# spvkgn/vorbis-aotuv-lancer

Measured on AMD Instinct MI355X. Metric: realtime-stream-equivalents/node (44.1kHz stereo q5) + MDCT HBM GB/s, higher is better.
Workload: dtype f32

## Files before the change

vorbis_aotuv_lancer_amd/csrc/capi_frontend.cpp:

```cpp
#include <hip/hip_runtime.h>
#include <stdio.h>
#include <string.h>
#include <string>
#include <vector>

#include "vorbis_mi355x.h"
#include "setup_host.h"
#include "frontend.h"
#include "frontend_kernels.h"
#include "mdct_kernel.h"
#include "kernels.h"
#include "vbm_internal.h"

struct vbm_frontend {
    vbm_encoder *enc;
    vbm_setup_host *H;
    const vbm_setup *hs;
    int S, ch;
    vbm_fe_state f;
    std::vector<void *> allocs;
    vbm_fe_decision *d_dec = nullptr, *h_dec = nullptr;
    int *d_ids = nullptr, *d_begin = nullptr;
    int *h_ids = nullptr, *h_begin = nullptr;
    uint8_t *h_flags = nullptr;
    vbm_fe_job *d_jobs = nullptr, *h_jobs = nullptr;
    uint8_t *d_hold = nullptr, *h_hold = nullptr;
    bool hold_active = false;
    float *d_blocks = nullptr;
    int blocks_turn = 0, nblocks_bufs = 2;
    std::vector<int> pcm_current, W, started, ended;
    hipStream_t q = nullptr;
    hipEvent_t ev_in = nullptr, ev_out = nullptr;
    int lane0[4] = {0, 0, 0, 0}, lane_cap[4] = {0, 0, 0, 0}, lanes = 0;
    signed char *d_type = nullptr;
    int *d_slot = nullptr, *d_begin_lane = nullptr;
    unsigned long long *d_stats = nullptr;
    float *d_blocks_dev = nullptr;
    std::vector<long long> written;
    bool mirrors_stale = false;
    bool dirty = false;
    int pending_steps = 0;
};

template <typename T>
static int fe_alloc(vbm_frontend *fe, T **p, size_t count)
{
    hipError_t err = hipMalloc((void **)p, count * sizeof(T) + 256);
    if (err != hipSuccess) return vbm_set_hip_error(err, "hipMalloc(front end)");
    fe->allocs.push_back(*p);
// ... 57 lines not shown
    f.base_max = (int)(bs1 * (cap_blocks / 3));
    f.plane = (long)S * ch * f.cap;
    f.marks = (int)(f.cap / 64) + 8;
    int rc = 0;
#define A(field, type, count) do { type *p_; rc = fe_alloc<type>(fe, &p_, (count)); if (rc) { vbm_frontend_destroy(fe); return rc; } field = p_; } while (0)
    const size_t SC = (size_t)S * ch;
    A(f.pcm, float, (size_t)2 * f.plane);
    A(f.parity, int, S);
    A(f.base, int, S);
    A(f.overflow, int, 1);
    A(f.pcm_current, int, S); A(f.centerW, int, S); A(f.lW, int, S); A(f.W, int, S); A(f.nW, int, S);
    A(f.eofflag, int, S); A(f.preextrapolate, int, S);
    A(f.granulepos, long long, S); A(f.sequence, long long, S);
    A(f.ve_current, int, S); A(f.ve_cursor, int, S); A(f.ve_curmark, int, S); A(f.ve_stretch, int, S);
    A(f.ve_mark, int, (size_t)f.marks * S);
    A(f.ve_ampbuf, float, (size_t)16 * VBM_VE_AMP * SC);
    A(f.ve_ampptr, int, (size_t)16 * SC);
    A(f.ve_nearDC, float, (size_t)VBM_VE_NEARDC * SC);
    A(f.ve_nearacc, float, (size_t)2 * SC);
    A(f.ve_nearptr, int, SC);
    A(f.ve_first, int, S); A(f.ve_last, int, S);
    A(f.ve_spec, float, SC * VBM_FE_CHUNK * 64);
    A(fe->d_dec, vbm_fe_decision, S);
    A(fe->d_ids, int, S); A(fe->d_begin, int, S);
    fe->nblocks_bufs = vbm_encoder_workspaces(enc);
    A(fe->d_blocks, float, (size_t)fe->nblocks_bufs * SC * bs1);
    A(fe->d_hold, uint8_t, (size_t)S);
    if (hipHostMalloc((void **)&fe->h_hold, (size_t)S, hipHostMallocDefault) != hipSuccess) {
        vbm_frontend_destroy(fe);
        g_vbm_err = "hipHostMalloc(hold mask) failed";
// ... 31 lines not shown
    if (!fe) return VBM_EINVAL;
    const vbm_fe_state &f = fe->f;
    const int S = fe->S, bs1 = fe->hs->blocksizes[1];
    const size_t SC = (size_t)S * fe->ch;
    hipError_t err = hipDeviceSynchronize();
    auto zero = [&](void *p, size_t bytes) { if (err == hipSuccess) err = hipMemset(p, 0, bytes); };
    zero(f.pcm, (size_t)2 * f.plane * sizeof(float));
    zero(f.parity, S * sizeof(int));
    zero(f.base, S * sizeof(int));
    zero(f.overflow, sizeof(int));
    zero(f.lW, S * sizeof(int)); zero(f.W, S * sizeof(int)); zero(f.nW, S * sizeof(int));
    zero(f.eofflag, S * sizeof(int)); zero(f.preextrapolate, S * sizeof(int));
    zero(f.granulepos, S * sizeof(long long));
    zero(f.ve_current, S * sizeof(int)); zero(f.ve_stretch, S * sizeof(int));
    zero(f.ve_mark, (size_t)f.marks * S * sizeof(int));
    zero(f.ve_ampbuf, (size_t)16 * VBM_VE_AMP * SC * sizeof(float));
    zero(f.ve_ampptr, (size_t)16 * SC * sizeof(int));
    zero(f.ve_nearDC, (size_t)VBM_VE_NEARDC * SC * sizeof(float));
    zero(f.ve_nearacc, 2 * SC * sizeof(float));
    zero(f.ve_nearptr, SC * sizeof(int));
    if (err != hipSuccess) return vbm_set_hip_error(err, "hipMemset(front end)");
    std::vector<int> half(S, bs1 / 2), minus1(S, -1);
    std::vector<long long> seq(S, 3);
    if ((err = hipMemcpy(f.pcm_current, half.data(), S * sizeof(int), hipMemcpyHostToDevice)) != hipSuccess ||
        (err = hipMemcpy(f.centerW, half.data(), S * sizeof(int), hipMemcpyHostToDevice)) != hipSuccess ||
        (err = hipMemcpy(f.ve_cursor, half.data(), S * sizeof(int), hipMemcpyHostToDevice)) != hipSuccess ||
        (err = hipMemcpy(f.ve_curmark, minus1.data(), S * sizeof(int), hipMemcpyHostToDevice)) != hipSuccess ||
        (err = hipMemcpy(f.sequence, seq.data(), S * sizeof(long long), hipMemcpyHostToDevice)) != hipSuccess)
        return vbm_set_hip_error(err, "hipMemcpy(front end init)");
    fe->pcm_current.assign(S, bs1 / 2);
// ... 305 lines not shown
    }
    if ((err = hipMemcpyAsync(fe->d_ids, fe->h_ids, total * sizeof(int), hipMemcpyHostToDevice, st)) != hipSuccess ||
        (err = hipMemcpyAsync(fe->d_begin, fe->h_begin, total * sizeof(int), hipMemcpyHostToDevice, st)) != hipSuccess)
        return vbm_set_hip_error(err, "hipMemcpyAsync(round lists)");

    {
        int rc = vbm_analysis_round_wait_workspace(fe->enc, fq);
        if (rc) return rc;
    }
    float *round_blocks = fe->d_blocks + (size_t)fe->blocks_turn * S * ch * bs1;
    fe->blocks_turn = (fe->blocks_turn + 1) % fe->nblocks_bufs;
    for (int m = 0; m < 4; m++) {
        if (!count[m]) continue;
        const int N = (m >> 1) ? bs1 : bs0;
        float *blocks = round_blocks + (size_t)offset[m] * ch * bs1;
        if (vbm_fe_launch_gather(&fe->f, fe->d_ids + offset[m], fe->d_begin + offset[m], count[m], N, blocks, nullptr, st))
            return VBM_EHIP;
    }
    vbm_debug_delay_point(VBM_DP_FE_FORK, st);
    {
        int rc = vbm_analysis_round_begin(fe->enc, count, fe->h_ids, fe->h_flags, round_blocks, d_packets, d_packet_bytes, fq);
        if (rc) return rc;
        if (!defer && (rc = vbm_analysis_round_join(fe->enc, stream))) return rc;
    }
    vbm_debug_delay_point(VBM_DP_FE_SHIFT, st);
    if (vbm_fe_launch_shift(&fe->f, fe->d_dec, st)) return VBM_EHIP;
    *nblocks = total;
    return VBM_OK;
}

extern "C" int vbm_frontend_encode_round(vbm_frontend *fe, uint8_t *d_packets, int *d_packet_bytes,
// ... 138 lines not shown
{
    if (!fe || nrounds < 1 || !d_packet_bytes || !d_info || !d_counts) return VBM_EINVAL;
    const vbm_setup *s = fe->hs;
    const vbm_setup *ds = vbm_setup_device(fe->H);
    const int S = fe->S, ch = fe->ch, bs0 = s->blocksizes[0], bs1 = s->blocksizes[1];
    const int maxb = vbm_encoder_max_packet_bytes(fe->enc);
    hipStream_t q = fe->q;
    hipError_t err;
    int rc = fe_enter(fe, stream);
    if (rc) return rc;
    vbm_debug_stamp(q, 1);
    if (!fe->lanes) {
        lane_layout(s, S, fe->lane0, fe->lane_cap, &fe->lanes);
        const size_t L = (size_t)fe->lanes;
#define A(field, type, count) do { type *p_; rc = fe_alloc<type>(fe, &p_, (count)); if (rc) return rc; field = p_; } while (0)
        A(fe->d_type, signed char, (size_t)S);
        A(fe->d_slot, int, (size_t)S);
        A(fe->d_begin_lane, int, L);
        A(fe->d_stats, unsigned long long, 8);
        A(fe->d_blocks_dev, float, (size_t)fe->nblocks_bufs * L * ch * bs1);
#undef A
        if ((err = hipDeviceSynchronize()) != hipSuccess) return vbm_set_hip_error(err, "hipDeviceSynchronize");
    }
    if (fe_evaluate_envelope(fe, q)) return VBM_EHIP;
    for (int r = 0; r < nrounds; r++) {
        int w, ws_lanes;
        int *d_sid, *counts_ws;
        uint8_t *d_wf;
        rc = vbm_encoder_device_round_open(fe->enc, q, &w, &d_sid, &d_wf, &ws_lanes, &counts_ws);
        if (rc) return rc;
        if (ws_lanes < fe->lanes) {
            g_vbm_err = "encoder workspace too small for rounds built on the device: create it with max_batch >= vbm_device_round_lanes()";
            return VBM_EINVAL;
        }
        float *blocks = fe->d_blocks_dev + (size_t)w * fe->lanes * ch * bs1;
        int *counts_r = d_counts + 4 * r;
        int *bytes_r = d_packet_bytes + (size_t)r * fe->lanes;
        int caps[4];
        for (int m = 0; m < 4; m++) caps[m] = fe->lane_cap[m];
        if (r > 0 && caps[2] > 0 && caps[3] > 2 * caps[2]) caps[3] = 2 * caps[2];
        vbm_fe_round R;
        for (int m = 0; m < 4; m++) { R.lane0[m] = fe->lane0[m]; R.cap[m] = caps[m]; }
        R.first_round = r == 0;
        R.count = counts_ws;
        R.slot = fe->d_slot;
        R.stream_id = d_sid;
        R.wflags = d_wf;
        R.begin = fe->d_begin_lane;
        R.info = d_info + (size_t)r * fe->lanes;
        R.stats = fe->d_stats;
        vbm_debug_delay_point(VBM_DP_DEV_PLAN, q);
        if (vbm_fe_launch_round_plan(&fe->f, ds, &R, fe->d_type, fe->d_dec, bytes_r, fe->lanes, q)) return VBM_EHIP;
        if ((err = hipMemcpyAsync(counts_r, counts_ws, 4 * sizeof(int), hipMemcpyDeviceToDevice, q)) != hipSuccess)
            return vbm_set_hip_error(err, "hipMemcpyAsync(counts)");
        for (int m = 0; m < 4; m++) {
            if (!caps[m]) continue;
            const int N = (m >> 1) ? bs1 : bs0;
            if (vbm_fe_launch_gather(&fe->f, d_sid + fe->lane0[m], fe->d_begin_lane + fe->lane0[m], caps[m], N,
                                     blocks + (size_t)fe->lane0[m] * ch * bs1, counts_ws + m, q))
                return VBM_EHIP;
        }
        vbm_debug_stamp(q, 2 + (r ? 1 : 0));
        rc = vbm_encoder_device_round_run(fe->enc, w, fe->lane0, caps, counts_ws, blocks,
                                          d_packets ? d_packets + (size_t)r * fe->lanes * maxb : nullptr, bytes_r, r == 0, q);
        if (rc) return rc;
        vbm_debug_delay_point(VBM_DP_FE_SHIFT, q);
        if (vbm_fe_launch_shift(&fe->f, fe->d_dec, q)) return VBM_EHIP;
    }
    vbm_debug_stamp(q, 4);
    fe->mirrors_stale = true;
    if (lazy == 2) return VBM_OK;
    return lazy ? vbm_analysis_round_join_lazy(fe->enc, stream) : vbm_analysis_round_join(fe->enc, stream);
}

extern "C" int vbm_frontend_round_types(vbm_frontend *fe, signed char *out, void *stream)
{
    if (!fe || !out || !fe->d_type) return VBM_EINVAL;
    hipError_t err = hipMemcpyAsync(out, fe->d_type, (size_t)fe->S, hipMemcpyDeviceToHost, (hipStream_t)stream);
    return err == hipSuccess ? VBM_OK : vbm_set_hip_error(err, "hipMemcpyAsync(round types)");
}

extern "C" int vbm_frontend_device_stats(vbm_frontend *fe, unsigned long long *out)
{
    if (!fe || !out) return VBM_EINVAL;
    for (int i = 0; i < 6; i++) out[i] = 0;
    hipError_t err;
    int ov = 0;
    if ((err = hipStreamSynchronize(fe->q)) != hipSuccess ||
        (err = hipMemcpy(&ov, fe->f.overflow, sizeof(int), hipMemcpyDeviceToHost)) != hipSuccess)
        return vbm_set_hip_error(err, "hipMemcpy(stats)");
    out[5] = (unsigned long long)ov;
    if (!fe->d_stats) return VBM_OK;
    if ((err = hipMemcpy(out, fe->d_stats, 5 * sizeof(unsigned long long), hipMemcpyDeviceToHost)) != hipSuccess)
        return vbm_set_hip_error(err, "hipMemcpy(stats)");
    return VBM_OK;
}

extern "C" int vbm_debug_poison_frontend(vbm_frontend *fe, int byte)
{
    if (!fe) return VBM_EINVAL;
    hipError_t err = hipDeviceSynchronize();
    if (err != hipSuccess) return vbm_set_hip_error(err, "hipDeviceSynchronize");
    const size_t SC = (size_t)fe->S * fe->ch, bs1 = (size_t)fe->hs->blocksizes[1];
    if ((err = hipMemset(fe->d_blocks, byte, (size_t)fe->nblocks_bufs * SC * bs1 * sizeof(float))) != hipSuccess ||
        (err = hipMemset(fe->f.ve_spec, byte, SC * VBM_FE_CHUNK * 64 * sizeof(float))) != hipSuccess ||
        (err = hipMemset(fe->d_ids, byte, (size_t)fe->S * sizeof(int))) != hipSuccess ||
        (err = hipMemset(fe->d_begin, byte, (size_t)fe->S * sizeof(int))) != hipSuccess ||
        (fe->d_blocks_dev && (err = hipMemset(fe->d_blocks_dev, byte, (size_t)fe->nblocks_bufs * fe->lanes * fe->ch * bs1 * sizeof(float))) != hipSuccess) ||
        (fe->d_begin_lane && (err = hipMemset(fe->d_begin_lane, byte, (size_t)fe->lanes * sizeof(int))) != hipSuccess))
        return vbm_set_hip_error(err, "hipMemset(poison)");
    err = hipDeviceSynchronize();
    return err == hipSuccess ? VBM_OK : vbm_set_hip_error(err, "hipDeviceSynchronize");
}

extern "C" int vbm_frontend_join(vbm_frontend *fe, void *stream)
{
    if (!fe) return VBM_EINVAL;
    return vbm_analysis_round_join(fe->enc, stream);
}
```

vorbis_aotuv_lancer_amd/csrc/frontend.h:

```cpp
#pragma once
#include <stdint.h>
#include "setup.h"
#include "vorbis_mi355x.h"

#define VBM_FE_CHUNK 32

struct vbm_fe_state {
    int S, ch;
    long cap;
    long plane;
    int marks;
    float *pcm;
    int *parity;
    int *base;
    int base_max;
    int *overflow;
    int *pcm_current, *centerW, *lW, *W, *nW, *eofflag, *preextrapolate;
    long long *granulepos, *sequence;
    int *ve_current, *ve_cursor, *ve_curmark, *ve_stretch;
    int *ve_mark;
    float *ve_ampbuf;
    int *ve_ampptr;
    float *ve_nearDC;
    float *ve_nearacc;
    int *ve_nearptr;
    int *ve_first, *ve_last;
    float *ve_spec;
};

struct vbm_fe_job {
    long long src;
    long long ch_stride;
    int stream, vals;
};

struct vbm_fe_decision {
    int ready;
    int lW, W, nW;
    int block_mode;
    int eos;
    int beginW;
    int movement;
    long long granulepos, sequence;
};

struct vbm_fe_round {
    int lane0[4], cap[4];
    int first_round;
    int *count;
    int *slot;
    int *stream_id;
    uint8_t *wflags;
    int *begin;
    vbm_packet_info *info;
    unsigned long long *stats;
};
```

vorbis_aotuv_lancer_amd/csrc/frontend_kernels.h:

```cpp
#pragma once
#include <hip/hip_runtime.h>
#include "frontend.h"

extern "C" {
int vbm_fe_launch_append(const vbm_fe_state *f, const float *d_src, int vals, float pre_amplitude, hipStream_t st);
int vbm_fe_launch_append_ids(const vbm_fe_state *f, const int *d_ids, int n, const float *d_src, int vals,
                             float pre_amplitude, long stream_stride, long ch_stride, int by_slot, hipStream_t st);
int vbm_fe_launch_append_ragged(const vbm_fe_state *f, const vbm_fe_job *d_jobs, int n, int max_vals, const float *d_src,
                                float pre_amplitude, hipStream_t st);
int vbm_fe_launch_restart(const vbm_fe_state *f, const int *d_ids, int n, int long_n, hipStream_t st);
int vbm_fe_launch_extrapolate(const vbm_fe_state *f, const int *d_ids, int nids, int mode, int long_n, hipStream_t st);
int vbm_fe_launch_ve_range(const vbm_fe_state *f, hipStream_t st);
int vbm_fe_launch_ve_filter(const vbm_fe_state *f, const vbm_setup *d_setup, int t0, hipStream_t st);
int vbm_fe_launch_decide(const vbm_fe_state *f, const vbm_setup *d_setup, vbm_fe_decision *d_out, const uint8_t *d_hold,
                         hipStream_t st);
int vbm_fe_launch_gather(const vbm_fe_state *f, const int *d_ids, const int *d_begin, int count, int N, float *d_dst,
                         const int *d_count, hipStream_t st);
int vbm_fe_launch_round_plan(const vbm_fe_state *f, const vbm_setup *d_setup, const vbm_fe_round *r, signed char *d_type,
                             vbm_fe_decision *d_dec, int *d_packet_bytes, int lanes, hipStream_t st);
int vbm_fe_launch_shift(const vbm_fe_state *f, const vbm_fe_decision *d_dec, hipStream_t st);
}
```

vorbis_aotuv_lancer_amd/csrc/frontend_kernels.hip:

```cpp
#include <hip/hip_runtime.h>
#include <stdint.h>
#include "batch.h"
#include "frontend.h"
#include "frontend_kernels.h"

namespace {

__device__ __forceinline__ float *chan_buf(const vbm_fe_state &f, int s, int c)
{
    return f.pcm + (long)f.parity[s] * f.plane + ((long)s * f.ch + c) * f.cap + f.base[s];
}

__device__ __forceinline__ bool fe_full(const vbm_fe_state &f, int s, int vals)
{
    return f.base[s] + f.pcm_current[s] + vals > f.cap;
}

__device__ __forceinline__ void fe_append_one(const vbm_fe_state &f, int s, int c, const float *in, int vals,
                                              float pre_amplitude)
{
    if (fe_full(f, s, vals)) return;
    float *dst = f.pcm + (long)f.parity[s] * f.plane + (long)(s * f.ch + c) * f.cap + f.base[s] + f.pcm_current[s];
    const int t0 = blockIdx.y * blockDim.x + threadIdx.x, step = gridDim.y * blockDim.x;
    if ((((uintptr_t)dst | (uintptr_t)in) & 15) == 0 && (vals & 3) == 0) {
// ... 68 lines not shown
    float *pcm = f.pcm + (long)f.parity[s] * f.plane + c * f.cap;
    for (int i = 0; i < long_n / 2; i++) pcm[i] = 0.f;
    for (int k = 0; k < VBM_VE_AMP; k++)
        for (int jb = 0; jb < 16; jb++) f.ve_ampbuf[((long)k * SC + c) * 16 + jb] = 0.f;
    for (int jb = 0; jb < 16; jb++) f.ve_ampptr[c * 16 + jb] = 0;
    for (int k = 0; k < VBM_VE_NEARDC; k++) f.ve_nearDC[(long)k * SC + c] = 0.f;
    f.ve_nearacc[c] = 0.f;
    f.ve_nearacc[SC + c] = 0.f;
    f.ve_nearptr[c] = 0;
    if (ci == 0) {
        f.base[s] = 0;
        f.pcm_current[s] = long_n / 2; f.centerW[s] = long_n / 2;
        f.lW[s] = 0; f.W[s] = 0; f.nW[s] = 0; f.eofflag[s] = 0; f.preextrapolate[s] = 0;
        f.granulepos[s] = 0; f.sequence[s] = 3;
        f.ve_current[s] = 0; f.ve_cursor[s] = long_n / 2; f.ve_curmark[s] = -1; f.ve_stretch[s] = 0;
        for (int k = 0; k < f.marks; k++) f.ve_mark[(long)k * f.S + s] = 0;
    }
}

template <int M, typename Acc>
__device__ void lpc_from_data(Acc data, float *lpci, int n)
{
    double aut[M + 1], lpc[M];
    double error, epsilon;
    int i, j;

    j = M + 1;
    while (j--) {
        double d = 0;
        for (i = j; i < n; i++) d += (double)data(i) * (double)data(i - j);
        aut[j] = d;
// ... 122 lines not shown
__global__ __launch_bounds__(64) void k_fe_ve_filter(vbm_fe_state f, const vbm_setup *__restrict__ setup, int t0)
{
    __shared__ float s_vec[4][32];
    extern __shared__ float s_ring[];
    const int grp = threadIdx.x >> 4, jb = threadIdx.x & 15;
    const int s = blockIdx.x * 4 + grp;
    if (s >= f.S) return;
    const vbm_envelope *ve = &setup->ve;
    const long SC = (long)f.S * f.ch;
    const int first = f.ve_first[s] + t0, last = f.ve_last[s];
    if (first >= last) return;
    const int ch = f.ch;
    const float minV = ve->minenergy;
    const float stretch_penalty = ve->stretch_penalty;
    int ve_stretch = f.ve_stretch[s];
    const int S = f.S;
    const bool band = jb < VBM_VE_BANDS;
    const int begin = band ? ve->band_begin[jb] : 0, end = band ? ve->band_end[jb] : 0;
    const float total = band ? ve->band_total[jb] : 0.f;
    const float pre_t = band ? ve->preecho_thresh[jb] : 0.f, post_t = band ? ve->postecho_thresh[jb] : 0.f;
    float bw[VBM_VE_MAXBAND];
#pragma unroll
    for (int i = 0; i < VBM_VE_MAXBAND; i++) bw[i] = band ? ve->band_window[jb][i] : 0.f;

    constexpr int PER_CH = VBM_VE_AMP * 16 + 16 + 16 + 4;
    float *R = s_ring + (size_t)grp * ch * PER_CH;
    for (int ci = 0; ci < ch; ci++) {
        const long c = (long)s * ch + ci;
        float *rc = R + ci * PER_CH;
#pragma unroll
        for (int k = 0; k < VBM_VE_AMP; k++) rc[k * 16 + jb] = f.ve_ampbuf[((long)k * SC + c) * 16 + jb];
// ... 130 lines not shown

            if (valmax > pre_t + penalty) ret |= 1 | 4;
            if (valmin < post_t - penalty) ret |= 2;
        }
        __builtin_amdgcn_fence(__ATOMIC_RELEASE, "wavefront");
        __builtin_amdgcn_wave_barrier();
        __builtin_amdgcn_fence(__ATOMIC_ACQUIRE, "wavefront");

        if (ci == ch - 1) {
            ret |= __builtin_amdgcn_update_dpp(0, ret, 0xB1, 0xf, 0xf, true);
            ret |= __builtin_amdgcn_update_dpp(0, ret, 0x4E, 0xf, 0xf, true);
            ret |= __builtin_amdgcn_update_dpp(0, ret, 0x141, 0xf, 0xf, true);
            ret |= __builtin_amdgcn_update_dpp(0, ret, 0x140, 0xf, 0xf, true);

            if (jb == 0) {
                f.ve_mark[(long)(j + VBM_VE_POST) * S + s] = 0;
                if (ret & 1) {
                    f.ve_mark[(long)j * S + s] = 1;
                    f.ve_mark[(long)(j + 1) * S + s] = 1;
                }
                if (ret & 2) {
                    f.ve_mark[(long)j * S + s] = 1;
                    if (j > 0) f.ve_mark[(long)(j - 1) * S + s] = 1;
                }
            }
            if (ret & 4) ve_stretch = -1;
        }
    }
    if (jb == 0) {
        f.ve_stretch[s] = ve_stretch;
        if (first + nsteps >= last) f.ve_current[s] = last * 64;
    }

    for (int ci = 0; ci < ch; ci++) {
        const long c = (long)s * ch + ci;
        const float *rc = R + ci * PER_CH;
#pragma unroll
        for (int k = 0; k < VBM_VE_AMP; k++) f.ve_ampbuf[((long)k * SC + c) * 16 + jb] = rc[k * 16 + jb];
// ... 8 lines not shown
    }
}

__device__ __forceinline__ vbm_fe_decision fe_no_decision()
{
    vbm_fe_decision d;
    d.ready = 0; d.lW = d.W = d.nW = 0; d.block_mode = 0; d.eos = 0; d.beginW = 0; d.movement = 0;
    d.granulepos = 0; d.sequence = 0;
    return d;
}

template <bool COMMIT>
__device__ __forceinline__ void fe_decide_one(const vbm_fe_state &f, const vbm_setup *__restrict__ setup, const int s,
                                              vbm_fe_decision &d)
{
    const int S = f.S;
    const int searchstep = 64;
    const int bs0 = setup->blocksizes[0], bs1 = setup->blocksizes[1];
    d = fe_no_decision();

    int W = f.W[s], lW = f.lW[s], nW = f.nW[s];
    int centerW = f.centerW[s], pcm_current = f.pcm_current[s], eofflag = f.eofflag[s];
    const int bsW = W ? bs1 : bs0;
    const int beginW = centerW - bsW / 2;

    if (!f.preextrapolate[s] || eofflag == -1) return;

    int bp = -1;
    int curmark;
    {
        const int ve_current = (pcm_current / searchstep - VBM_VE_WIN) * searchstep;
        if (COMMIT) f.ve_current[s] = ve_current;
        const int testW = centerW + bsW / 4 + bs1 / 2 + bs0 / 4;
        int j = f.ve_cursor[s];
        int cursor = j;
        curmark = f.ve_curmark[s];
        while (j < ve_current - searchstep) {
            if (j >= testW) { bp = 1; break; }
            cursor = j;
            if (f.ve_mark[(long)(j / searchstep) * S + s]) {
                if (j > centerW) {
                    curmark = j;
                    bp = (j >= testW) ? 1 : 0;
                    break;
                }
            }
            j += searchstep;
        }
        if (COMMIT) {
            f.ve_cursor[s] = cursor;
            f.ve_curmark[s] = curmark;
        }
    }

    if (bp == -1) {
// ... 12 lines not shown
    }

    d.ready = 1;
    d.lW = lW; d.W = W; d.nW = nW;
    int blocktype;
    if (W) {
        blocktype = (!lW || !nW) ? 0  : 1 ;
    } else {
        int b0 = centerW - bs0 / 4 - bs0 / 4;
        int e0 = centerW + bs0 / 4 + bs0 / 4;
        int marked = 0;
        if (curmark >= b0 && curmark < e0) marked = 1;
        else {
            const int first = b0 / searchstep, last = e0 / searchstep;
            for (int i = first; i < last; i++)
                if (f.ve_mark[(long)i * S + s]) { marked = 1; break; }
        }
        blocktype = marked ? 0  : 1 ;
    }
    d.block_mode = blocktype | (W << 1);
    if (!COMMIT) return;
    d.sequence = f.sequence[s]++;
    long long granulepos = f.granulepos[s];
    d.granulepos = granulepos;
    d.beginW = beginW;

    if (eofflag) {
        if (centerW >= eofflag) {
            f.eofflag[s] = -1;
            d.eos = 1;
            return;
        }
    }

    {
        const int new_centerNext = bs1 / 2;
        const int movementW = centerNext - new_centerNext;
        if (movementW > 0) {
            {
                int ve_current = f.ve_current[s];
                const int smallsize = ve_current / searchstep + VBM_VE_POST;
                const int smallshift = movementW / searchstep;
                for (int k = 0; k < smallsize - smallshift; k++)
                    f.ve_mark[(long)k * S + s] = f.ve_mark[(long)(k + smallshift) * S + s];
                f.ve_current[s] = ve_current - movementW;
                int cm = f.ve_curmark[s];
                if (cm >= 0) f.ve_curmark[s] = cm - movementW;
                f.ve_cursor[s] -= movementW;
            }
            pcm_current -= movementW;
            f.pcm_current[s] = pcm_current;
            d.movement = movementW;

            f.lW[s] = W;
            f.W[s] = nW;
            f.centerW[s] = new_centerNext;
            centerW = new_centerNext;

            if (eofflag) {
// ... 9 lines not shown
        }
    }
}

__global__ void k_fe_decide(vbm_fe_state f, const vbm_setup *__restrict__ setup, vbm_fe_decision *__restrict__ out,
                            const uint8_t *__restrict__ hold)
{
    const int s = blockIdx.x * blockDim.x + threadIdx.x;
    if (s >= f.S) return;
    vbm_fe_decision d;
    if (hold && hold[s]) d = fe_no_decision();
    else fe_decide_one<true>(f, setup, s, d);
    out[s] = d;
}

__global__ void k_fe_classify(vbm_fe_state f, const vbm_setup *__restrict__ setup, signed char *__restrict__ type)
{
    const int s = blockIdx.x * blockDim.x + threadIdx.x;
    if (s >= f.S) return;
    vbm_fe_decision d;
    d.ready = 0;
    fe_decide_one<false>(f, setup, s, d);
    type[s] = d.ready ? (signed char)(d.block_mode & 3) : (signed char)-1;
}

__global__ __launch_bounds__(1024) void k_fe_plan(vbm_fe_round r, const signed char *__restrict__ type, int S)
{
    __shared__ int s_part[16][4];
    __shared__ int s_carry[4];
    const int lane = threadIdx.x & 63, wave = threadIdx.x >> 6;
    if (threadIdx.x < 4) s_carry[threadIdx.x] = 0;
    __syncthreads();
    for (int base = 0; base < S; base += 1024) {
        const int s = base + threadIdx.x;
        const int t = s < S ? type[s] : -1;
        int incl[4], mine[4];
#pragma unroll
        for (int m = 0; m < 4; m++) {
            mine[m] = (t == m) ? 1 : 0;
            int v = mine[m];
#pragma unroll
            for (int d = 1; d < 64; d <<= 1) {
                const int u = __shfl_up(v, d);
                if (lane >= d) v += u;
            }
            incl[m] = v;
            if (lane == 63) s_part[wave][m] = v;
        }
        __syncthreads();
        if (s < S) {
            int slot = -1;
            if (t >= 0) {
                int before = s_carry[t];
                for (int w = 0; w < wave; w++) before += s_part[w][t];
                const int rank = before + incl[t] - 1;
                if (rank < r.cap[t]) slot = r.lane0[t] + rank;
            }
            r.slot[s] = slot;
        }
        __syncthreads();
        if (threadIdx.x < 4) {
            int tot = s_carry[threadIdx.x];
            for (int w = 0; w < 16; w++) tot += s_part[w][threadIdx.x];
            s_carry[threadIdx.x] = tot;
        }
        __syncthreads();
    }
    if (threadIdx.x < 4) {
        const int m = threadIdx.x;
        const int n = s_carry[m] < r.cap[m] ? s_carry[m] : r.cap[m];
        r.count[m] = n;
        atomicAdd(&r.stats[m], (unsigned long long)n);
    }
}

__global__ void k_fe_round_commit(vbm_fe_state f, const vbm_setup *__restrict__ setup, vbm_fe_round r,
                                  vbm_fe_decision *__restrict__ dec)
{
    const int s = blockIdx.x * blockDim.x + threadIdx.x;
    if (s >= f.S) return;
    vbm_fe_decision d = fe_no_decision();
    const int slot = r.slot[s];
    if (slot >= 0) {
        fe_decide_one<true>(f, setup, s, d);
        r.stream_id[slot] = s;
        r.wflags[slot] = (uint8_t)(d.lW | (d.nW << 1));
        r.begin[slot] = d.beginW;
        vbm_packet_info pi;
        pi.stream = s; pi.block_mode = d.block_mode; pi.lW = d.lW; pi.W = d.W; pi.nW = d.nW; pi.eos = d.eos;
        pi.granulepos = d.granulepos; pi.packetno = d.sequence;
        r.info[slot] = pi;
        if (d.movement > 0) atomicAdd(&r.stats[4], (unsigned long long)d.movement);
    }
    dec[s] = d;
}

__global__ void k_fe_blank(vbm_fe_round r, int *__restrict__ packet_bytes, int lanes)
{
    const int k = blockIdx.x * blockDim.x + threadIdx.x;
    if (k >= lanes) return;
    int m = 3;
#pragma unroll
    for (int t = 0; t < 4; t++)
        if (k >= r.lane0[t] && k < r.lane0[t] + r.cap[t]) m = t;
    const bool inside = k >= r.lane0[m] && k < r.lane0[m] + r.cap[m];
    if (!inside || k - r.lane0[m] >= r.count[m]) {
        r.info[k].stream = -1;
        packet_bytes[k] = -2;
    }
}

__global__ void k_fe_gather(vbm_fe_state f, const int *__restrict__ ids, const int *__restrict__ begin, int count,
                            int N, float *__restrict__ dst, const int *__restrict__ d_count)
{
    const int kc = blockIdx.x;
    const int k = kc / f.ch, c = kc % f.ch;
    if (d_count) count = *d_count;
    if (k >= count) return;
    const int s = ids[k];
    const float4 *src = reinterpret_cast<const float4 *>(chan_buf(f, s, c) + begin[k]);
    float4 *out = reinterpret_cast<float4 *>(dst + ((long)k * f.ch + c) * N);
    for (int i = blockIdx.y * blockDim.x + threadIdx.x; i < N / 4; i += gridDim.y * blockDim.x) out[i] = src[i];
}

__global__ void k_fe_shift(vbm_fe_state f, const vbm_fe_decision *__restrict__ dec)
{
    const int c = blockIdx.x;
    const int s = c / f.ch;
    const int mv = dec[s].movement;
    if (mv <= 0) return;
    const int nb = f.base[s] + mv;
    if (nb <= f.base_max) return;
    const int n = f.pcm_current[s];
    const int par = f.parity[s];
    const float4 *src = reinterpret_cast<const float4 *>(f.pcm + (long)par * f.plane + (long)c * f.cap + nb);
    float4 *dst = reinterpret_cast<float4 *>(f.pcm + (long)(par ^ 1) * f.plane + (long)c * f.cap);
    for (int i = blockIdx.y * blockDim.x + threadIdx.x; i < (n + 3) / 4; i += gridDim.y * blockDim.x) dst[i] = src[i];
}

__global__ void k_fe_flip(vbm_fe_state f, const vbm_fe_decision *__restrict__ dec)
{
    const int s = blockIdx.x * blockDim.x + threadIdx.x;
    if (s >= f.S) return;
    const int mv = dec[s].movement;
    if (mv <= 0) return;
    const int nb = f.base[s] + mv;
    if (nb > f.base_max) {
        f.parity[s] ^= 1;
        f.base[s] = 0;
    } else {
        f.base[s] = nb;
    }
}

}

#define CHECK_LAUNCH() (hipGetLastError() == hipSuccess ? 0 : -2)

extern "C" int vbm_fe_launch_append(const vbm_fe_state *f, const float *d_src, int vals, float pre_amplitude, hipStream_t st)
{
    const unsigned gx = (unsigned)((vals + 1023) / 1024);
    hipLaunchKernelGGL(k_fe_append, dim3((unsigned)(f->S * f->ch), gx ? gx : 1), dim3(256), 0, st, *f, d_src, vals, pre_amplitude);
    hipLaunchKernelGGL(k_fe_commit, dim3((unsigned)((f->S + 255) / 256)), dim3(256), 0, st, *f, vals);
    return CHECK_LAUNCH();
}

// ... 45 lines not shown
{
    const size_t lds = (size_t)4 * f->ch * (VBM_VE_AMP * 16 + 16 + 16 + 4) * sizeof(float);
    if (lds > 60 * 1024) return -2;
    hipLaunchKernelGGL(k_fe_ve_filter, dim3((unsigned)((f->S + 3) / 4)), dim3(64), lds, st, *f, d_setup, t0);
    return CHECK_LAUNCH();
}

extern "C" int vbm_fe_launch_decide(const vbm_fe_state *f, const vbm_setup *d_setup, vbm_fe_decision *d_out,
                                    const uint8_t *d_hold, hipStream_t st)
{
    hipLaunchKernelGGL(k_fe_decide, dim3((unsigned)((f->S + 63) / 64)), dim3(64), 0, st, *f, d_setup, d_out, d_hold);
    return CHECK_LAUNCH();
}

extern "C" int vbm_fe_launch_gather(const vbm_fe_state *f, const int *d_ids, const int *d_begin, int count, int N,
                                    float *d_dst, const int *d_count, hipStream_t st)
{
    if (count <= 0) return 0;
    hipLaunchKernelGGL(k_fe_gather, dim3((unsigned)(count * f->ch), (unsigned)((N / 4 + 255) / 256)), dim3(256), 0, st, *f,
                       d_ids, d_begin, count, N, d_dst, d_count);
    return CHECK_LAUNCH();
}

extern "C" int vbm_fe_launch_round_plan(const vbm_fe_state *f, const vbm_setup *d_setup, const vbm_fe_round *r,
                                        signed char *d_type, vbm_fe_decision *d_dec, int *d_packet_bytes, int lanes,
                                        hipStream_t st)
{
    const dim3 g((unsigned)((f->S + 63) / 64));
    hipLaunchKernelGGL(k_fe_classify, g, dim3(64), 0, st, *f, d_setup, d_type);
    hipLaunchKernelGGL(k_fe_plan, dim3(1), dim3(1024), 0, st, *r, d_type, f->S);
    hipLaunchKernelGGL(k_fe_round_commit, g, dim3(64), 0, st, *f, d_setup, *r, d_dec);
    hipLaunchKernelGGL(k_fe_blank, dim3((unsigned)((lanes + 255) / 256)), dim3(256), 0, st, *r, d_packet_bytes, lanes);
    return CHECK_LAUNCH();
}

extern "C" int vbm_fe_launch_shift(const vbm_fe_state *f, const vbm_fe_decision *d_dec, hipStream_t st)
{
    hipLaunchKernelGGL(k_fe_shift, dim3((unsigned)(f->S * f->ch), 4), dim3(256), 0, st, *f, d_dec);
    hipLaunchKernelGGL(k_fe_flip, dim3((unsigned)((f->S + 255) / 256)), dim3(256), 0, st, *f, d_dec);
    return CHECK_LAUNCH();
}
```

Measured before the change: 101,900.

## Fuse device round head: ring-buffer envelope marks, one-pass plan, merged gather and shift

Envelope marks become a ring buffer with a per-stream origin offset, so advancing no longer copies the whole mark array per stream. The plan kernel now gives each wave a contiguous span and ranks streams with ballot/popcount in two passes. It also writes stream ids, window flags, begin offsets, the count copy and lane blanking directly, which removes the separate blank kernel and the device-to-device count memcpy. The four per-mode gather launches become one lane-indexed gather kernel, and the shift and flip kernels are merged into one block per stream. The cost is less parallelism per stream in shift and gather, and more state to keep consistent.

```diff
diff --git a/vorbis_aotuv_lancer_amd/csrc/capi_frontend.cpp b/vorbis_aotuv_lancer_amd/csrc/capi_frontend.cpp
--- a/vorbis_aotuv_lancer_amd/csrc/capi_frontend.cpp
+++ b/vorbis_aotuv_lancer_amd/csrc/capi_frontend.cpp
@@ -32,7 +32,7 @@
     hipStream_t q = nullptr;
     hipEvent_t ev_in = nullptr, ev_out = nullptr;
     int lane0[4] = {0, 0, 0, 0}, lane_cap[4] = {0, 0, 0, 0}, lanes = 0;
-    signed char *d_type = nullptr;
+    vbm_fe_look look = {nullptr, nullptr, nullptr};
     int *d_slot = nullptr, *d_begin_lane = nullptr;
     unsigned long long *d_stats = nullptr;
     float *d_blocks_dev = nullptr;
@@ -120,6 +120,7 @@
     A(f.granulepos, long long, S); A(f.sequence, long long, S);
     A(f.ve_current, int, S); A(f.ve_cursor, int, S); A(f.ve_curmark, int, S); A(f.ve_stretch, int, S);
     A(f.ve_mark, int, (size_t)f.marks * S);
+    A(f.ve_org, int, S);
     A(f.ve_ampbuf, float, (size_t)16 * VBM_VE_AMP * SC);
     A(f.ve_ampptr, int, (size_t)16 * SC);
     A(f.ve_nearDC, float, (size_t)VBM_VE_NEARDC * SC);
@@ -181,6 +182,7 @@
     zero(f.granulepos, S * sizeof(long long));
     zero(f.ve_current, S * sizeof(int)); zero(f.ve_stretch, S * sizeof(int));
     zero(f.ve_mark, (size_t)f.marks * S * sizeof(int));
+    zero(f.ve_org, S * sizeof(int));
     zero(f.ve_ampbuf, (size_t)16 * VBM_VE_AMP * SC * sizeof(float));
     zero(f.ve_ampptr, (size_t)16 * SC * sizeof(int));
     zero(f.ve_nearDC, (size_t)VBM_VE_NEARDC * SC * sizeof(float));
@@ -516,7 +518,7 @@
         if (!count[m]) continue;
         const int N = (m >> 1) ? bs1 : bs0;
         float *blocks = round_blocks + (size_t)offset[m] * ch * bs1;
-        if (vbm_fe_launch_gather(&fe->f, fe->d_ids + offset[m], fe->d_begin + offset[m], count[m], N, blocks, nullptr, st))
+        if (vbm_fe_launch_gather(&fe->f, fe->d_ids + offset[m], fe->d_begin + offset[m], count[m], N, blocks, st))
             return VBM_EHIP;
     }
     vbm_debug_delay_point(VBM_DP_FE_FORK, st);
@@ -685,7 +687,9 @@
         lane_layout(s, S, fe->lane0, fe->lane_cap, &fe->lanes);
         const size_t L = (size_t)fe->lanes;
 #define A(field, type, count) do { type *p_; rc = fe_alloc<type>(fe, &p_, (count)); if (rc) return rc; field = p_; } while (0)
-        A(fe->d_type, signed char, (size_t)S);
+        A(fe->look.type, signed char, (size_t)S);
+        A(fe->look.wflags, uint8_t, (size_t)S);
+        A(fe->look.begin, int, (size_t)S);
         A(fe->d_slot, int, (size_t)S);
         A(fe->d_begin_lane, int, L);
         A(fe->d_stats, unsigned long long, 8);
@@ -712,8 +716,11 @@
         if (r > 0 && caps[2] > 0 && caps[3] > 2 * caps[2]) caps[3] = 2 * caps[2];
         vbm_fe_round R;
         for (int m = 0; m < 4; m++) { R.lane0[m] = fe->lane0[m]; R.cap[m] = caps[m]; }
+        R.lanes = fe->lanes;
         R.first_round = r == 0;
         R.count = counts_ws;
+        R.count_out = counts_r;
+        R.packet_bytes = bytes_r;
         R.slot = fe->d_slot;
         R.stream_id = d_sid;
         R.wflags = d_wf;
@@ -721,16 +728,7 @@
         R.info = d_info + (size_t)r * fe->lanes;
         R.stats = fe->d_stats;
         vbm_debug_delay_point(VBM_DP_DEV_PLAN, q);
-        if (vbm_fe_launch_round_plan(&fe->f, ds, &R, fe->d_type, fe->d_dec, bytes_r, fe->lanes, q)) return VBM_EHIP;
-        if ((err = hipMemcpyAsync(counts_r, counts_ws, 4 * sizeof(int), hipMemcpyDeviceToDevice, q)) != hipSuccess)
-            return vbm_set_hip_error(err, "hipMemcpyAsync(counts)");
-        for (int m = 0; m < 4; m++) {
-            if (!caps[m]) continue;
-            const int N = (m >> 1) ? bs1 : bs0;
-            if (vbm_fe_launch_gather(&fe->f, d_sid + fe->lane0[m], fe->d_begin_lane + fe->lane0[m], caps[m], N,
-                                     blocks + (size_t)fe->lane0[m] * ch * bs1, counts_ws + m, q))
-                return VBM_EHIP;
-        }
+        if (vbm_fe_launch_round_head(&fe->f, ds, &R, &fe->look, fe->d_dec, bs0, bs1, blocks, q)) return VBM_EHIP;
         vbm_debug_stamp(q, 2 + (r ? 1 : 0));
         rc = vbm_encoder_device_round_run(fe->enc, w, fe->lane0, caps, counts_ws, blocks,
                                           d_packets ? d_packets + (size_t)r * fe->lanes * maxb : nullptr, bytes_r, r == 0, q);
@@ -746,8 +744,8 @@
 
 extern "C" int vbm_frontend_round_types(vbm_frontend *fe, signed char *out, void *stream)
 {
-    if (!fe || !out || !fe->d_type) return VBM_EINVAL;
-    hipError_t err = hipMemcpyAsync(out, fe->d_type, (size_t)fe->S, hipMemcpyDeviceToHost, (hipStream_t)stream);
+    if (!fe || !out || !fe->look.type) return VBM_EINVAL;
+    hipError_t err = hipMemcpyAsync(out, fe->look.type, (size_t)fe->S, hipMemcpyDeviceToHost, (hipStream_t)stream);
     return err == hipSuccess ? VBM_OK : vbm_set_hip_error(err, "hipMemcpyAsync(round types)");
 }
 
@@ -778,7 +776,9 @@
         (err = hipMemset(fe->d_ids, byte, (size_t)fe->S * sizeof(int))) != hipSuccess ||
         (err = hipMemset(fe->d_begin, byte, (size_t)fe->S * sizeof(int))) != hipSuccess ||
         (fe->d_blocks_dev && (err = hipMemset(fe->d_blocks_dev, byte, (size_t)fe->nblocks_bufs * fe->lanes * fe->ch * bs1 * sizeof(float))) != hipSuccess) ||
-        (fe->d_begin_lane && (err = hipMemset(fe->d_begin_lane, byte, (size_t)fe->lanes * sizeof(int))) != hipSuccess))
+        (fe->d_begin_lane && (err = hipMemset(fe->d_begin_lane, byte, (size_t)fe->lanes * sizeof(int))) != hipSuccess) ||
+        (fe->look.type && ((err = hipMemset(fe->look.wflags, byte, (size_t)fe->S)) != hipSuccess ||
+                           (err = hipMemset(fe->look.begin, byte, (size_t)fe->S * sizeof(int))) != hipSuccess)))
         return vbm_set_hip_error(err, "hipMemset(poison)");
     err = hipDeviceSynchronize();
     return err == hipSuccess ? VBM_OK : vbm_set_hip_error(err, "hipDeviceSynchronize");
diff --git a/vorbis_aotuv_lancer_amd/csrc/frontend.h b/vorbis_aotuv_lancer_amd/csrc/frontend.h
--- a/vorbis_aotuv_lancer_amd/csrc/frontend.h
+++ b/vorbis_aotuv_lancer_amd/csrc/frontend.h
@@ -19,6 +19,7 @@
     long long *granulepos, *sequence;
     int *ve_current, *ve_cursor, *ve_curmark, *ve_stretch;
     int *ve_mark;
+    int *ve_org;
     float *ve_ampbuf;
     int *ve_ampptr;
     float *ve_nearDC;
@@ -44,10 +45,19 @@
     long long granulepos, sequence;
 };
 
+struct vbm_fe_look {
+    signed char *type;
+    uint8_t *wflags;
+    int *begin;
+};
+
 struct vbm_fe_round {
     int lane0[4], cap[4];
+    int lanes;
     int first_round;
     int *count;
+    int *count_out;
+    int *packet_bytes;
     int *slot;
     int *stream_id;
     uint8_t *wflags;
diff --git a/vorbis_aotuv_lancer_amd/csrc/frontend_kernels.h b/vorbis_aotuv_lancer_amd/csrc/frontend_kernels.h
--- a/vorbis_aotuv_lancer_amd/csrc/frontend_kernels.h
+++ b/vorbis_aotuv_lancer_amd/csrc/frontend_kernels.h
@@ -15,8 +15,8 @@
 int vbm_fe_launch_decide(const vbm_fe_state *f, const vbm_setup *d_setup, vbm_fe_decision *d_out, const uint8_t *d_hold,
                          hipStream_t st);
 int vbm_fe_launch_gather(const vbm_fe_state *f, const int *d_ids, const int *d_begin, int count, int N, float *d_dst,
-                         const int *d_count, hipStream_t st);
-int vbm_fe_launch_round_plan(const vbm_fe_state *f, const vbm_setup *d_setup, const vbm_fe_round *r, signed char *d_type,
-                             vbm_fe_decision *d_dec, int *d_packet_bytes, int lanes, hipStream_t st);
+                         hipStream_t st);
+int vbm_fe_launch_round_head(const vbm_fe_state *f, const vbm_setup *d_setup, const vbm_fe_round *r, const vbm_fe_look *look,
+                             vbm_fe_decision *d_dec, int n_short, int n_long, float *d_blocks, hipStream_t st);
 int vbm_fe_launch_shift(const vbm_fe_state *f, const vbm_fe_decision *d_dec, hipStream_t st);
 }
diff --git a/vorbis_aotuv_lancer_amd/csrc/frontend_kernels.hip b/vorbis_aotuv_lancer_amd/csrc/frontend_kernels.hip
--- a/vorbis_aotuv_lancer_amd/csrc/frontend_kernels.hip
+++ b/vorbis_aotuv_lancer_amd/csrc/frontend_kernels.hip
@@ -3,8 +3,14 @@
 #include "batch.h"
 #include "frontend.h"
 #include "frontend_kernels.h"
+#include "round_head.h"
 
 namespace {
+
+__device__ __forceinline__ int &fe_mark(const vbm_fe_state &f, int s, int org, int k)
+{
+    return f.ve_mark[(long)fe_mark_row(org, k, f.marks) * f.S + s];
+}
 
 __device__ __forceinline__ float *chan_buf(const vbm_fe_state &f, int s, int c)
 {
@@ -106,7 +112,8 @@
         f.lW[s] = 0; f.W[s] = 0; f.nW[s] = 0; f.eofflag[s] = 0; f.preextrapolate[s] = 0;
         f.granulepos[s] = 0; f.sequence[s] = 3;
         f.ve_current[s] = 0; f.ve_cursor[s] = long_n / 2; f.ve_curmark[s] = -1; f.ve_stretch[s] = 0;
-        for (int k = 0; k < f.marks; k++) f.ve_mark[(long)k * f.S + s] = 0;
+        f.ve_org[s] = 0;
+        for (int k = 0; k < f.marks; k++) fe_mark(f, s, 0, k) = 0;
     }
 }
 
@@ -259,7 +266,7 @@
     const float minV = ve->minenergy;
     const float stretch_penalty = ve->stretch_penalty;
     int ve_stretch = f.ve_stretch[s];
-    const int S = f.S;
+    const int org = f.ve_org[s];
     const bool band = jb < VBM_VE_BANDS;
     const int begin = band ? ve->band_begin[jb] : 0, end = band ? ve->band_end[jb] : 0;
     const float total = band ? ve->band_total[jb] : 0.f;
@@ -420,14 +427,14 @@
             ret |= __builtin_amdgcn_update_dpp(0, ret, 0x140, 0xf, 0xf, true);
 
             if (jb == 0) {
-                f.ve_mark[(long)(j + VBM_VE_POST) * S + s] = 0;
+                fe_mark(f, s, org, j + VBM_VE_POST) = 0;
                 if (ret & 1) {
-                    f.ve_mark[(long)j * S + s] = 1;
-                    f.ve_mark[(long)(j + 1) * S + s] = 1;
+                    fe_mark(f, s, org, j) = 1;
+                    fe_mark(f, s, org, j + 1) = 1;
                 }
                 if (ret & 2) {
-                    f.ve_mark[(long)j * S + s] = 1;
-                    if (j > 0) f.ve_mark[(long)(j - 1) * S + s] = 1;
+                    fe_mark(f, s, org, j) = 1;
+                    if (j > 0) fe_mark(f, s, org, j - 1) = 1;
                 }
             }
             if (ret & 4) ve_stretch = -1;
@@ -466,9 +473,9 @@
 __device__ __forceinline__ void fe_decide_one(const vbm_fe_state &f, const vbm_setup *__restrict__ setup, const int s,
                                               vbm_fe_decision &d)
 {
-    const int S = f.S;
     const int searchstep = 64;
     const int bs0 = setup->blocksizes[0], bs1 = setup->blocksizes[1];
+    const int org = f.ve_org[s];
     d = fe_no_decision();
 
     int W = f.W[s], lW = f.lW[s], nW = f.nW[s];
@@ -490,7 +497,7 @@
         while (j < ve_current - searchstep) {
             if (j >= testW) { bp = 1; break; }
             cursor = j;
-            if (f.ve_mark[(long)(j / searchstep) * S + s]) {
+            if (fe_mark(f, s, org, j / searchstep)) {
                 if (j > centerW) {
                     curmark = j;
                     bp = (j >= testW) ? 1 : 0;
@@ -533,16 +540,16 @@
         else {
             const int first = b0 / searchstep, last = e0 / searchstep;
             for (int i = first; i < last; i++)
-                if (f.ve_mark[(long)i * S + s]) { marked = 1; break; }
+                if (fe_mark(f, s, org, i)) { marked = 1; break; }
         }
         blocktype = marked ? 0  : 1 ;
     }
     d.block_mode = blocktype | (W << 1);
+    d.beginW = beginW;
     if (!COMMIT) return;
     d.sequence = f.sequence[s]++;
     long long granulepos = f.granulepos[s];
     d.granulepos = granulepos;
-    d.beginW = beginW;
 
     if (eofflag) {
         if (centerW >= eofflag) {
@@ -558,10 +565,7 @@
         if (movementW > 0) {
             {
                 int ve_current = f.ve_current[s];
-                const int smallsize = ve_current / searchstep + VBM_VE_POST;
-                const int smallshift = movementW / searchstep;
-                for (int k = 0; k < smallsize - smallshift; k++)
-                    f.ve_mark[(long)k * S + s] = f.ve_mark[(long)(k + smallshift) * S + s];
+                f.ve_org[s] = fe_mark_advance(org, movementW / searchstep, f.marks);
                 f.ve_current[s] = ve_current - movementW;
                 int cm = f.ve_curmark[s];
                 if (cm >= 0) f.ve_curmark[s] = cm - movementW;
@@ -601,63 +605,103 @@
     out[s] = d;
 }
 
-__global__ void k_fe_classify(vbm_fe_state f, const vbm_setup *__restrict__ setup, signed char *__restrict__ type)
+__global__ void k_fe_classify(vbm_fe_state f, const vbm_setup *__restrict__ setup, vbm_fe_look look)
 {
     const int s = blockIdx.x * blockDim.x + threadIdx.x;
     if (s >= f.S) return;
     vbm_fe_decision d;
     d.ready = 0;
     fe_decide_one<false>(f, setup, s, d);
-    type[s] = d.ready ? (signed char)(d.block_mode & 3) : (signed char)-1;
-}
-
-__global__ __launch_bounds__(1024) void k_fe_plan(vbm_fe_round r, const signed char *__restrict__ type, int S)
+    look.type[s] = d.ready ? (signed char)(d.block_mode & 3) : (signed char)-1;
+    look.wflags[s] = (uint8_t)(d.lW | (d.nW << 1));
+    look.begin[s] = d.beginW;
+}
+
+__global__ __launch_bounds__(1024) void k_fe_plan(vbm_fe_round r, vbm_fe_look look, int S)
 {
     __shared__ int s_part[16][4];
-    __shared__ int s_carry[4];
     const int lane = threadIdx.x & 63, wave = threadIdx.x >> 6;
-    if (threadIdx.x < 4) s_carry[threadIdx.x] = 0;
+    const int span = fe_plan_span(S, 16);
+    const int s0 = wave * span, s1 = s0 + span < S ? s0 + span : S;
+    constexpr int NC = 8;
+    {
+        int tot[4] = {0, 0, 0, 0};
+        for (int b = s0; b < s1; b += 64 * NC) {
+            int tc[NC];
+#pragma unroll
+            for (int i = 0; i < NC; i++) {
+                const int s = b + 64 * i + lane;
+                tc[i] = s < s1 ? look.type[s] : -1;
+            }
+#pragma unroll
+            for (int i = 0; i < NC; i++)
+#pragma unroll
+                for (int m = 0; m < 4; m++) tot[m] += __popcll(__ballot(tc[i] == m));
+        }
+        if (lane < 4) s_part[wave][lane] = lane == 0 ? tot[0] : lane == 1 ? tot[1] : lane == 2 ? tot[2] : tot[3];
+    }
     __syncthreads();
-    for (int base = 0; base < S; base += 1024) {
-        const int s = base + threadIdx.x;
-        const int t = s < S ? type[s] : -1;
-        int incl[4], mine[4];
-#pragma unroll
-        for (int m = 0; m < 4; m++) {
-            mine[m] = (t == m) ? 1 : 0;
-            int v = mine[m];
-#pragma unroll
-            for (int d = 1; d < 64; d <<= 1) {
-                const int u = __shfl_up(v, d);
-                if (lane >= d) v += u;
-            }
-            incl[m] = v;
-            if (lane == 63) s_part[wave][m] = v;
-        }
-        __syncthreads();
-        if (s < S) {
-            int slot = -1;
-            if (t >= 0) {
-                int before = s_carry[t];
-                for (int w = 0; w < wave; w++) before += s_part[w][t];
-                const int rank = before + incl[t] - 1;
-                if (rank < r.cap[t]) slot = r.lane0[t] + rank;
-            }
-            r.slot[s] = slot;
-        }
-        __syncthreads();
-        if (threadIdx.x < 4) {
-            int tot = s_carry[threadIdx.x];
-            for (int w = 0; w < 16; w++) tot += s_part[w][threadIdx.x];
-            s_carry[threadIdx.x] = tot;
-        }
-        __syncthreads();
-    }
+    int before[4], total[4];
+#pragma unroll
+    for (int m = 0; m < 4; m++) {
+        before[m] = total[m] = 0;
+        for (int w = 0; w < 16; w++) {
+            const int v = s_part[w][m];
+            if (w < wave) before[m] += v;
+            total[m] += v;
+        }
+    }
+    for (int b = s0; b < s1; b += 64 * NC) {
+        int tc[NC], bc[NC];
+        uint8_t wc[NC];
+#pragma unroll
+        for (int i = 0; i < NC; i++) {
+            const int s = b + 64 * i + lane;
+            const bool in = s < s1;
+            tc[i] = in ? look.type[s] : -1;
+            wc[i] = in ? look.wflags[s] : 0;
+            bc[i] = in ? look.begin[s] : 0;
+        }
+#pragma unroll
+        for (int i = 0; i < NC; i++) {
+            if (b + 64 * i >= s1) break;
+            const int s = b + 64 * i + lane, t = tc[i];
+            int rank = 0, lane0 = 0, cap = 0;
+#pragma unroll
+            for (int m = 0; m < 4; m++) {
+                const uint64_t bm = __ballot(t == m);
+                if (t == m) { rank = before[m] + fe_plan_rank64(bm, lane); lane0 = r.lane0[m]; cap = r.cap[m]; }
+                before[m] += __popcll(bm);
+            }
+            if (s < s1) {
+                const int slot = t >= 0 ? fe_plan_slot(rank, lane0, cap) : -1;
+                r.slot[s] = slot;
+                if (slot >= 0) {
+                    r.stream_id[slot] = s;
+                    r.wflags[slot] = wc[i];
+                    r.begin[slot] = bc[i];
+                }
+            }
+        }
+    }
+    int n[4];
+#pragma unroll
+    for (int m = 0; m < 4; m++) n[m] = total[m] < r.cap[m] ? total[m] : r.cap[m];
     if (threadIdx.x < 4) {
         const int m = threadIdx.x;
-        const int n = s_carry[m] < r.cap[m] ? s_carry[m] : r.cap[m];
-        r.count[m] = n;
-        atomicAdd(&r.stats[m], (unsigned long long)n);
+        const int nm = m == 0 ? n[0] : m == 1 ? n[1] : m == 2 ? n[2] : n[3];
+        r.count[m] = nm;
+        r.count_out[m] = nm;
+        atomicAdd(&r.stats[m], (unsigned long long)nm);
+    }
+    for (int k = threadIdx.x; k < r.lanes; k += 1024) {
+        bool inside;
+        const int m = fe_lane_region(r.lane0, r.cap, k, &inside);
+        const int nm = m == 0 ? n[0] : m == 1 ? n[1] : m == 2 ? n[2] : n[3];
+        if (!inside || k - r.lane0[m] >= nm) {
+            r.info[k].stream = -1;
+            r.packet_bytes[k] = -2;
+        }
     }
 }
 
@@ -670,9 +714,6 @@
     const int slot = r.slot[s];
     if (slot >= 0) {
         fe_decide_one<true>(f, setup, s, d);
-        r.stream_id[slot] = s;
-        r.wflags[slot] = (uint8_t)(d.lW | (d.nW << 1));
-        r.begin[slot] = d.beginW;
         vbm_packet_info pi;
         pi.stream = s; pi.block_mode = d.block_mode; pi.lW = d.lW; pi.W = d.W; pi.nW = d.nW; pi.eos = d.eos;
         pi.granulepos = d.granulepos; pi.packetno = d.sequence;
@@ -682,27 +723,11 @@
     dec[s] = d;
 }
 
-__global__ void k_fe_blank(vbm_fe_round r, int *__restrict__ packet_bytes, int lanes)
-{
-    const int k = blockIdx.x * blockDim.x + threadIdx.x;
-    if (k >= lanes) return;
-    int m = 3;
-#pragma unroll
-    for (int t = 0; t < 4; t++)
-        if (k >= r.lane0[t] && k < r.lane0[t] + r.cap[t]) m = t;
-    const bool inside = k >= r.lane0[m] && k < r.lane0[m] + r.cap[m];
-    if (!inside || k - r.lane0[m] >= r.count[m]) {
-        r.info[k].stream = -1;
-        packet_bytes[k] = -2;
-    }
-}
-
 __global__ void k_fe_gather(vbm_fe_state f, const int *__restrict__ ids, const int *__restrict__ begin, int count,
-                            int N, float *__restrict__ dst, const int *__restrict__ d_count)
+                            int N, float *__restrict__ dst)
 {
     const int kc = blockIdx.x;
     const int k = kc / f.ch, c = kc % f.ch;
-    if (d_count) count = *d_count;
     if (k >= count) return;
     const int s = ids[k];
     const float4 *src = reinterpret_cast<const float4 *>(chan_buf(f, s, c) + begin[k]);
@@ -710,33 +735,64 @@
     for (int i = blockIdx.y * blockDim.x + threadIdx.x; i < N / 4; i += gridDim.y * blockDim.x) out[i] = src[i];
 }
 
-__global__ void k_fe_shift(vbm_fe_state f, const vbm_fe_decision *__restrict__ dec)
-{
-    const int c = blockIdx.x;
-    const int s = c / f.ch;
+__global__ __launch_bounds__(128) void k_fe_round_gather(vbm_fe_state f, vbm_fe_round r, int n_short, int n_long,
+                                                         long lane_stride, float *__restrict__ dst)
+{
+    const int kc = blockIdx.x;
+    const int lane = kc / f.ch, c = kc - lane * f.ch;
+    bool inside;
+    const int m = fe_lane_region(r.lane0, r.cap, lane, &inside);
+    if (!inside) return;
+    const int k = lane - r.lane0[m];
+    if (k >= r.count[m]) return;
+    const int N = (m >> 1) ? n_long : n_short;
+    const int s = r.stream_id[lane];
+    const float4 *src = reinterpret_cast<const float4 *>(chan_buf(f, s, c) + r.begin[lane]);
+    float4 *out = reinterpret_cast<float4 *>(dst + (long)r.lane0[m] * lane_stride + ((long)k * f.ch + c) * N);
+    const int n4 = N / 4;
+    for (int i = threadIdx.x; i < n4; i += 4 * 128) {
+        float4 v[4];
+#pragma unroll
+        for (int u = 0; u < 4; u++)
+            if (i + u * 128 < n4) v[u] = src[i + u * 128];
+#pragma unroll
+        for (int u = 0; u < 4; u++)
+            if (i + u * 128 < n4) out[i + u * 128] = v[u];
+    }
+}
+
+__global__ __launch_bounds__(256) void k_fe_shift(vbm_fe_state f, const vbm_fe_decision *__restrict__ dec)
+{
+    const int s = blockIdx.x;
     const int mv = dec[s].movement;
     if (mv <= 0) return;
     const int nb = f.base[s] + mv;
-    if (nb <= f.base_max) return;
-    const int n = f.pcm_current[s];
     const int par = f.parity[s];
-    const float4 *src = reinterpret_cast<const float4 *>(f.pcm + (long)par * f.plane + (long)c * f.cap + nb);
-    float4 *dst = reinterpret_cast<float4 *>(f.pcm + (long)(par ^ 1) * f.plane + (long)c * f.cap);
-    for (int i = blockIdx.y * blockDim.x + threadIdx.x; i < (n + 3) / 4; i += gridDim.y * blockDim.x) dst[i] = src[i];
-}
-
-__global__ void k_fe_flip(vbm_fe_state f, const vbm_fe_decision *__restrict__ dec)
-{
-    const int s = blockIdx.x * blockDim.x + threadIdx.x;
-    if (s >= f.S) return;
-    const int mv = dec[s].movement;
-    if (mv <= 0) return;
-    const int nb = f.base[s] + mv;
     if (nb > f.base_max) {
-        f.parity[s] ^= 1;
-        f.base[s] = 0;
-    } else {
-        f.base[s] = nb;
+        const int n4 = (f.pcm_current[s] + 3) / 4;
+        for (int c = 0; c < f.ch; c++) {
+            const long sc = (long)s * f.ch + c;
+            const float4 *src = reinterpret_cast<const float4 *>(f.pcm + (long)par * f.plane + sc * f.cap + nb);
+            float4 *dst = reinterpret_cast<float4 *>(f.pcm + (long)(par ^ 1) * f.plane + sc * f.cap);
+            for (int i = threadIdx.x; i < n4; i += 4 * 256) {
+                float4 v[4];
+#pragma unroll
+                for (int u = 0; u < 4; u++)
+                    if (i + u * 256 < n4) v[u] = src[i + u * 256];
+#pragma unroll
+                for (int u = 0; u < 4; u++)
+                    if (i + u * 256 < n4) dst[i + u * 256] = v[u];
+            }
+        }
+    }
+    __syncthreads();
+    if (threadIdx.x == 0) {
+        if (nb > f.base_max) {
+            f.parity[s] = par ^ 1;
+            f.base[s] = 0;
+        } else {
+            f.base[s] = nb;
+        }
     }
 }
 
@@ -812,29 +868,29 @@
 }
 
 extern "C" int vbm_fe_launch_gather(const vbm_fe_state *f, const int *d_ids, const int *d_begin, int count, int N,
-                                    float *d_dst, const int *d_count, hipStream_t st)
+                                    float *d_dst, hipStream_t st)
 {
     if (count <= 0) return 0;
     hipLaunchKernelGGL(k_fe_gather, dim3((unsigned)(count * f->ch), (unsigned)((N / 4 + 255) / 256)), dim3(256), 0, st, *f,
-                       d_ids, d_begin, count, N, d_dst, d_count);
-    return CHECK_LAUNCH();
-}
-
-extern "C" int vbm_fe_launch_round_plan(const vbm_fe_state *f, const vbm_setup *d_setup, const vbm_fe_round *r,
-                                        signed char *d_type, vbm_fe_decision *d_dec, int *d_packet_bytes, int lanes,
-                                        hipStream_t st)
+                       d_ids, d_begin, count, N, d_dst);
+    return CHECK_LAUNCH();
+}
+
+extern "C" int vbm_fe_launch_round_head(const vbm_fe_state *f, const vbm_setup *d_setup, const vbm_fe_round *r,
+                                        const vbm_fe_look *look, vbm_fe_decision *d_dec, int n_short, int n_long,
+                                        float *d_blocks, hipStream_t st)
 {
     const dim3 g((unsigned)((f->S + 63) / 64));
-    hipLaunchKernelGGL(k_fe_classify, g, dim3(64), 0, st, *f, d_setup, d_type);
-    hipLaunchKernelGGL(k_fe_plan, dim3(1), dim3(1024), 0, st, *r, d_type, f->S);
+    hipLaunchKernelGGL(k_fe_classify, g, dim3(64), 0, st, *f, d_setup, *look);
+    hipLaunchKernelGGL(k_fe_plan, dim3(1), dim3(1024), 0, st, *r, *look, f->S);
     hipLaunchKernelGGL(k_fe_round_commit, g, dim3(64), 0, st, *f, d_setup, *r, d_dec);
-    hipLaunchKernelGGL(k_fe_blank, dim3((unsigned)((lanes + 255) / 256)), dim3(256), 0, st, *r, d_packet_bytes, lanes);
+    hipLaunchKernelGGL(k_fe_round_gather, dim3((unsigned)(r->lanes * f->ch)), dim3(128), 0, st, *f, *r, n_short, n_long,
+                       (long)f->ch * n_long, d_blocks);
     return CHECK_LAUNCH();
 }
 
 extern "C" int vbm_fe_launch_shift(const vbm_fe_state *f, const vbm_fe_decision *d_dec, hipStream_t st)
 {
-    hipLaunchKernelGGL(k_fe_shift, dim3((unsigned)(f->S * f->ch), 4), dim3(256), 0, st, *f, d_dec);
-    hipLaunchKernelGGL(k_fe_flip, dim3((unsigned)((f->S + 255) / 256)), dim3(256), 0, st, *f, d_dec);
-    return CHECK_LAUNCH();
-}
+    hipLaunchKernelGGL(k_fe_shift, dim3((unsigned)f->S), dim3(256), 0, st, *f, d_dec);
+    return CHECK_LAUNCH();
+}
diff --git a/vorbis_aotuv_lancer_amd/csrc/round_head.h b/vorbis_aotuv_lancer_amd/csrc/round_head.h
--- /dev/null
+++ b/vorbis_aotuv_lancer_amd/csrc/round_head.h
@@ -0,0 +1,49 @@
+#pragma once
+#include <stdint.h>
+
+#ifdef __HIPCC__
+#define RH_FN __host__ __device__ __forceinline__
+#else
+#define RH_FN static inline
+#endif
+
+RH_FN int fe_mark_row(const int org, const int k, const int marks)
+{
+    const int p = org + k;
+    return p >= marks ? p - marks : p < 0 ? p + marks : p;
+}
+
+RH_FN int fe_mark_advance(const int org, const int steps, const int marks)
+{
+    return (int)(((long long)org + steps) % marks);
+}
+
+RH_FN int fe_plan_span(const int S, const int waves)
+{
+    const int groups = (S + 63) / 64;
+    return ((groups + waves - 1) / waves) * 64;
+}
+
+RH_FN int fe_plan_rank64(const uint64_t ballot, const int lane)
+{
+    const uint64_t below = ballot & ((1ull << lane) - 1ull);
+#ifdef __HIP_DEVICE_COMPILE__
+    return __popcll(below);
+#else
+    return __builtin_popcountll(below);
+#endif
+}
+
+RH_FN int fe_plan_slot(const int rank, const int lane0, const int cap)
+{
+    return rank < cap ? lane0 + rank : -1;
+}
+
+RH_FN int fe_lane_region(const int *lane0, const int *cap, const int k, bool *inside)
+{
+    int m = 3;
+    for (int t = 0; t < 4; t++)
+        if (k >= lane0[t] && k < lane0[t] + cap[t]) m = t;
+    *inside = k >= lane0[m] && k < lane0[m] + cap[m];
+    return m;
+}
```

New measurement: 101,200. No clear change (-0.7%).
